# polimi-ispl/deep_prior_interpolation

Hardware: AMD Instinct MI355X
Metric: Adam iters/sec on 3D MultiRes-UNet (whole job over n_gpus; per_gpu beside it); recon SNR(dB) vs ref under config.snr_vs_reference (higher is better)
Workload: dtype f32

## Files before the change

### deep_prior_interpolation_amd/csrc/elementwise.hip

```cpp
#include "common.h"
#include <stdlib.h>

namespace {

constexpr int kStatSpan = 16384;
constexpr int kMaxStatBlocks = 2048;

__host__ __device__ inline size_t stat_span(size_t V, int nblk) {
  size_t s = (V + nblk - 1) / nblk;
  return (s + 3) & ~(size_t)3;
}

typedef float ew_f32x4 __attribute__((ext_vector_type(4)));
constexpr size_t kNtMinFloats = (size_t)32 << 20;
__device__ __forceinline__ float4 ld4(const float* p, bool nt) {
  if (nt) { const ew_f32x4 v = __builtin_nontemporal_load(reinterpret_cast<const ew_f32x4*>(p)); return make_float4(v[0], v[1], v[2], v[3]); }
  return *reinterpret_cast<const float4*>(p);
}
__device__ __forceinline__ void st4(float* p, float4 v, bool nt) {
  if (nt) __builtin_nontemporal_store((ew_f32x4){v.x, v.y, v.z, v.w}, reinterpret_cast<ew_f32x4*>(p));
  else *reinterpret_cast<float4*>(p) = v;
}

template <bool xb = false>
// ... 425 lines not shown
      const float4 t = dpi_ld4(xa, i, tb, nt);
      const float4 u = dpi_ld4(xb, i, tb, nt);
      gv[0] = g.x; gv[1] = g.y; gv[2] = g.z; gv[3] = g.w;
      av[0] = t.x; av[1] = t.y; av[2] = t.z; av[3] = t.w;
      bv[0] = u.x; bv[1] = u.y; bv[2] = u.z; bv[3] = u.w;
    } else {
#pragma unroll
      for (int j = 0; j < 4; ++j) {
        const bool in = i + j < end;
        gv[j] = in ? dpi_ld(gc, i + j, gb) : 0.f; av[j] = in ? dpi_ld(xa, i + j, tb) : 0.f; bv[j] = in ? dpi_ld(xb, i + j, tb) : 0.f;
      }
    }
    float lsf = 0.f, lqf = 0.f;
#pragma unroll
    for (int j = 0; j < 4; ++j) {
      float xh, g;
      bn_bwd_elem(ka, av[j], gv[j], xh, g);
      ra[j] = ka.a * (g - a1 - xh * a2);
      bn_bwd_elem(kb, bv[j], gv[j], xh, g);
      rb[j] = dpi_stored(kb.a * (g - b1 - xh * b2), gb);
      if (forked && i + j < end) { float h, gf_; bn_bwd_elem(kf, bv[j], rb[j], h, gf_); lsf += gf_; lqf = fmaf(gf_, h, lqf); }
    }
    if (vec) {
      dpi_st4(oa, i, make_float4(ra[0], ra[1], ra[2], ra[3]), gb, nt);
      dpi_st4(ob, i, make_float4(rb[0], rb[1], rb[2], rb[3]), gb, nt);
    } else {
      for (int j = 0; j < 4 && i + j < end; ++j) { dpi_st(oa, i + j, ra[j], gb); dpi_st(ob, i + j, rb[j], gb); }
    }
    sf += lsf; qf += lqf;
  }
  if (f_partials && f_hi > f_lo) {
    __shared__ double sh[8];
    const double SF = block_sum(sf, sh), QF = block_sum(qf, sh + 4);
    if (threadIdx.x == 0 && forked) {
      f_partials[((size_t)b * fC + fc) * 2 + 0] = SF;
      f_partials[((size_t)b * fC + fc) * 2 + 1] = QF;
    }
  }
}

template <bool fb = false>
__global__ __launch_bounds__(256) void chain_add_apply_kernel(const float* __restrict__ a, const float* __restrict__ chain_a,
                                                              const float* __restrict__ b, const float* __restrict__ chain_b,
                                                              const float* __restrict__ chain_out, size_t V, float* __restrict__ y) {
  const bool nt = (size_t)gridDim.y * V >= kNtMinFloats;
  const int c = blockIdx.y;
  const Chain ta = load_chain(chain_a, c), tb = load_chain(chain_b, c), to = load_chain(chain_out, c);
  const float* __restrict__ ac = dpi_at(a, (size_t)c * V, fb);
  const float* __restrict__ bc = dpi_at(b, (size_t)c * V, fb);
  float* __restrict__ yc = dpi_at(y, (size_t)c * V, fb);
  const bool vec = (V & 3) == 0;
  for (size_t i = ((size_t)blockIdx.x * 256 + threadIdx.x) * 4; i < V; i += (size_t)gridDim.x * 1024) {
    if (vec) {
      const float4 f = dpi_ld4(ac, i, fb, nt), g = dpi_ld4(bc, i, fb, nt);
      float4 o;
      o.x = apply_chain(to, apply_chain(ta, f.x) + apply_chain(tb, g.x)); o.y = apply_chain(to, apply_chain(ta, f.y) + apply_chain(tb, g.y));
      o.z = apply_chain(to, apply_chain(ta, f.z) + apply_chain(tb, g.z)); o.w = apply_chain(to, apply_chain(ta, f.w) + apply_chain(tb, g.w));
      dpi_st4(yc, i, o, fb, nt);
    } else {
      for (int j = 0; j < 4 && i + j < V; ++j)
        dpi_st(yc, i + j, apply_chain(to, apply_chain(ta, dpi_ld(ac, i + j, fb)) + apply_chain(tb, dpi_ld(bc, i + j, fb))), fb);
    }
  }
}

constexpr int kJoinSums = 24;
constexpr int kJoinGroups = 2;
struct JoinSide {
  const float* x;
  const float* mean_invstd;
  const float* gamma;
  const float* beta;
  const float* in_chain;
  float post;
  const float* fwd_chain;
};
struct JoinFork {
  int lo, hi;
  const float* mean_invstd;
  const float* gamma;
  const float* beta;
  float post;
};
template <bool fb = false, bool gb = false>
__global__ __launch_bounds__(256) void join_bwd_sums_kernel(const float* __restrict__ dy, const float* __restrict__ t,
                                                            const float* __restrict__ mean_invstd, const float* __restrict__ gamma,
                                                            const float* __restrict__ beta, float pre, JoinSide A, JoinSide B, JoinFork F,
                                                            int C, size_t V, int nblk, double* __restrict__ partials) {
  const bool nt = (size_t)gridDim.y * V >= kNtMinFloats;
  const int c = blockIdx.y, b = blockIdx.x;
  const BnBwd k = bn_bwd_consts(mean_invstd, gamma, beta, nullptr, pre, 1.f, C, c);
  const BnBwd ka = bn_bwd_consts(A.mean_invstd, A.gamma, A.beta, A.in_chain, 1.f, A.post, C, c);
  const BnBwd kb = bn_bwd_consts(B.mean_invstd, B.gamma, B.beta, B.in_chain, 1.f, B.post, C, c);
  const bool forked = c >= F.lo && c < F.hi;
  const int fC = F.hi - F.lo, fc = forked ? c - F.lo : 0;
  const BnBwd kf = forked ? bn_bwd_consts(F.mean_invstd, F.gamma, F.beta, nullptr, 1.f, F.post, fC, fc) : ka;
  const size_t span = stat_span(V, nblk);
  const size_t beg = (size_t)b * span, end = beg + span < V ? beg + span : V;
  const float* __restrict__ gc = dpi_at(dy, (size_t)c * V, gb);
  const float* __restrict__ tc = t ? dpi_at(t, (size_t)c * V, fb) : nullptr;
  const float* __restrict__ xa = dpi_at(A.x, (size_t)c * V, fb);
  const float* __restrict__ xb = dpi_at(B.x, (size_t)c * V, fb);
  const Chain fwa = load_chain(A.fwd_chain, c), fwb = load_chain(B.fwd_chain, c);
  double s[kJoinSums];
#pragma unroll
  for (int i = 0; i < kJoinSums; ++i) s[i] = 0.0;
  const bool vec = (V & 3) == 0;
  for (size_t i0 = beg + (size_t)threadIdx.x * 4; i0 < end; i0 += 1024 * kJoinGroups) {
   float l[kJoinSums];
#pragma unroll
   for (int q = 0; q < kJoinSums; ++q) l[q] = 0.f;
#pragma unroll
   for (int u = 0; u < kJoinGroups; ++u) {
    const size_t i = i0 + (size_t)u * 1024;
    if (i >= end) break;
    float gv[4], tv[4], av[4], bv[4];
    if (vec) {
      const float4 g = dpi_ld4(gc, i, gb, nt), p = dpi_ld4(xa, i, fb, nt), q = dpi_ld4(xb, i, fb, nt);
      gv[0] = g.x; gv[1] = g.y; gv[2] = g.z; gv[3] = g.w;
      av[0] = p.x; av[1] = p.y; av[2] = p.z; av[3] = p.w;
      bv[0] = q.x; bv[1] = q.y; bv[2] = q.z; bv[3] = q.w;
      if (tc) { const float4 u = dpi_ld4(tc, i, fb, nt); tv[0] = u.x; tv[1] = u.y; tv[2] = u.z; tv[3] = u.w; }
    } else {
#pragma unroll
      for (int j = 0; j < 4; ++j) {
        const bool in = i + j < end;
        gv[j] = in ? dpi_ld(gc, i + j, gb) : 0.f; tv[j] = (in && tc) ? dpi_ld(tc, i + j, fb) : 0.f;
        av[j] = in ? dpi_ld(xa, i + j, fb) : 0.f; bv[j] = in ? dpi_ld(xb, i + j, fb) : 0.f;
      }
    }
    if (!tc) {
#pragma unroll
      for (int j = 0; j < 4; ++j) tv[j] = apply_chain(fwa, av[j]) + apply_chain(fwb, bv[j]);
    }
#pragma unroll
    for (int j = 0; j < 4; ++j)
      if (i + j < end) {
        float X, D, Xa, ma, Xb, mb;
        bn_bwd_elem(k, tv[j], gv[j], X, D);
        bn_bwd_elem(ka, av[j], 1.f, Xa, ma);
        bn_bwd_elem(kb, bv[j], 1.f, Xb, mb);
        const float P = (k.pre == 1.f || tv[j] > 0.f) ? k.a : k.a * k.pre;
        l[0] += D; l[1] = fmaf(D, X, l[1]);
        const float wa = ma * P, wb = mb * P;
        const float waD = wa * D, waX = wa * X, wbD = wb * D, wbX = wb * X;
        l[2] += waD; l[3] += wa; l[4] += waX;
        l[5] = fmaf(waD, Xa, l[5]); l[6] = fmaf(wa, Xa, l[6]); l[7] = fmaf(waX, Xa, l[7]);
        l[8] += wbD; l[9] += wb; l[10] += wbX;
        l[11] = fmaf(wbD, Xb, l[11]); l[12] = fmaf(wb, Xb, l[12]); l[13] = fmaf(wbX, Xb, l[13]);
        if (forked) {
          float Xf, mf;
          bn_bwd_elem(kf, bv[j], 1.f, Xf, mf);
          const float wf = mf * wb, wfD = wf * D, wfX = wf * X, mfXf = mf * Xf;
          l[14] += wfD; l[15] += wf; l[16] += wfX; l[17] += mf; l[18] = fmaf(mf, Xb, l[18]);
          l[19] = fmaf(wfD, Xf, l[19]); l[20] = fmaf(wf, Xf, l[20]); l[21] = fmaf(wfX, Xf, l[21]); l[22] += mfXf; l[23] = fmaf(mfXf, Xb, l[23]);
        }
      }
   }
#pragma unroll
   for (int q = 0; q < kJoinSums; ++q) s[q] += (double)l[q];
  }
  __shared__ double sh[4][kJoinSums];
  const int lane = threadIdx.x & 63, wid = threadIdx.x >> 6;
#pragma unroll
  for (int i = 0; i < kJoinSums; ++i) {
    const double v = wave_sum(s[i]);
// ... 303 lines not shown
          reinterpret_cast<unsigned*>(reinterpret_cast<unsigned short*>(yc) + o)[0] = dpi_pack_bf16(r0, r1);
        } else {
          if (2 * w < Wo) dpi_st(yc, o, r0, yb);
          if (2 * w + 1 < Wo) dpi_st(yc, o + 1, r1, yb);
        }
      }
    }
  }
}


template <bool SCALE_D, bool gb = false>
__global__ __launch_bounds__(256) void upsample_lin_bwd_gather_kernel(const float* __restrict__ dy, int D, int H, int W, int Do, int Ho,
                                                                      int Wo, float* __restrict__ dx) {
  const int c = blockIdx.y;
  const size_t V = (size_t)D * H * W, Vo = (size_t)Do * Ho * Wo;
  const float* __restrict__ gc = dpi_at(dy, (size_t)c * Vo, gb);
  float* __restrict__ oc = dpi_at(dx, (size_t)c * V, gb);
  for (size_t i = (size_t)blockIdx.x * 256 + threadIdx.x; i < V; i += (size_t)gridDim.x * 256) {
    const int w = i % W, h = (i / W) % H, d = i / ((size_t)W * H);
    int ow[4], oh[4], od[4];
    float ww[4], wh[4], wd[4];
    lin_bwd_taps(w, W, Wo, ow, ww);
    lin_bwd_taps(h, H, Ho, oh, wh);
    if (SCALE_D) lin_bwd_taps(d, D, Do, od, wd);
    float acc = 0.f;
#pragma unroll
    for (int a = 0; a < (SCALE_D ? 4 : 1); ++a) {
      const int od_ = SCALE_D ? od[a] : d;
      const float wa = SCALE_D ? wd[a] : 1.f;
      float accd = 0.f;
#pragma unroll
      for (int b = 0; b < 4; ++b) {
        const size_t row = ((size_t)od_ * Ho + oh[b]) * Wo;
        const float rsum = ww[0] * dpi_ld(gc, row + ow[0], gb) + ww[1] * dpi_ld(gc, row + ow[1], gb) + ww[2] * dpi_ld(gc, row + ow[2], gb)
                           + ww[3] * dpi_ld(gc, row + ow[3], gb);
        accd = fmaf(wh[b], rsum, accd);
      }
      acc = fmaf(wa, accd, acc);
    }
    dpi_st(oc, i, acc, gb);
  }
}

template <bool ib = false, bool ob = false>
__global__ __launch_bounds__(256) void upsample_lin_bwd_axis_kernel(const float* __restrict__ in, float* __restrict__ out, unsigned outer,
                                                                    int n, int no, unsigned inner) {
  const unsigned slab = (unsigned)n * inner;
  const unsigned per = slab < 256 ? 256 / slab : 1;
  const unsigned sub = per > 1 ? threadIdx.x / slab : 0;
  const unsigned e = per > 1 ? threadIdx.x - sub * slab : blockIdx.x * 256 + threadIdx.x;
  if (e >= slab || sub >= per) return;
  const unsigned i = e / inner, in_i = e - i * inner;
  int oo[4];
  float wt[4];
  lin_bwd_taps((int)i, n, no, oo, wt);
  const unsigned o0 = oo[0] * inner + in_i, o1 = oo[1] * inner + in_i, o2 = oo[2] * inner + in_i, o3 = oo[3] * inner + in_i;
  for (unsigned o = blockIdx.y * per + sub; o < outer; o += gridDim.y * per) {
    const float* __restrict__ p = dpi_at(in, (size_t)o * no * inner, ib);
    dpi_st(out, (size_t)o * slab + e, (wt[0] * dpi_ld(p, o0, ib) + wt[1] * dpi_ld(p, o1, ib)) + (wt[2] * dpi_ld(p, o2, ib) + wt[3] * dpi_ld(p, o3, ib)), ob);
  }
}

__global__ __launch_bounds__(256) void upsample_lin_bwd_w2_kernel(const float* __restrict__ in, float* __restrict__ out, size_t rows, int n) {
  const int half = n >> 1, no = 2 * n;
  const size_t total = rows * (size_t)half;
  for (size_t p = (size_t)blockIdx.x * 256 + threadIdx.x; p < total; p += (size_t)gridDim.x * 256) {
    const size_t r = p / half;
    const int i = 2 * (int)(p - r * half);
    const float* __restrict__ row = in + r * no;
    const float4 v = *reinterpret_cast<const float4*>(row + 2 * i);
    const float lo = row[i > 0 ? 2 * i - 1 : 0], hi = row[i + 1 < n - 1 ? 2 * i + 4 : 0];
    int o[4];
    float w0[4], w1[4];
    lin_bwd_taps(i, n, no, o, w0);
    lin_bwd_taps(i + 1, n, no, o, w1);
    float2 y;
    y.x = (w0[0] * lo + w0[1] * v.x) + (w0[2] * v.y + w0[3] * v.z);
    y.y = (w1[0] * v.y + w1[1] * v.z) + (w1[2] * v.w + w1[3] * hi);
    *reinterpret_cast<float2*>(out + r * n + i) = y;
  }
}

__global__ __launch_bounds__(256) void crop_copy_kernel(const float* __restrict__ x, int D, int H, int W, int od, int oh, int ow,
                                                        int Do, int Ho, int Wo, float* __restrict__ y, int adjoint) {
  const int c = blockIdx.y;
  const size_t V = (size_t)D * H * W, Vo = (size_t)Do * Ho * Wo;
  if (!adjoint) {
    for (size_t i = (size_t)blockIdx.x * 256 + threadIdx.x; i < Vo; i += (size_t)gridDim.x * 256) {
      const int w = i % Wo, h = (i / Wo) % Ho, d = i / ((size_t)Wo * Ho);
      y[(size_t)c * Vo + i] = x[(size_t)c * V + ((size_t)(d + od) * H + h + oh) * W + w + ow];
    }
  } else {
    for (size_t i = (size_t)blockIdx.x * 256 + threadIdx.x; i < V; i += (size_t)gridDim.x * 256) {
      const int w = i % W, h = (i / W) % H, d = i / ((size_t)W * H);
      const int cd = d - od, ch = h - oh, cw = w - ow;
      const bool in = cd >= 0 && cd < Do && ch >= 0 && ch < Ho && cw >= 0 && cw < Wo;
      y[(size_t)c * V + i] = in ? x[(size_t)c * Vo + ((size_t)cd * Ho + ch) * Wo + cw] : 0.f;
    }
  }
}

__global__ __launch_bounds__(256) void fir_axis0_kernel(const float* __restrict__ x, const float* __restrict__ taps, int K, int T, size_t S,
                                                        float* __restrict__ y) {
  const int c = blockIdx.y, p = K / 2;
  const size_t n = (size_t)T * S;
  for (size_t i = (size_t)blockIdx.x * 256 + threadIdx.x; i < n; i += (size_t)gridDim.x * 256) {
    const int t = (int)(i / S);
    const size_t s_ = i % S;
    float acc = 0.f;
    for (int k = 0; k < K; ++k) {
      const int tt = t + p - k;
      if (tt >= 0 && tt < T) acc = fmaf(taps[k], x[(size_t)c * n + (size_t)tt * S + s_], acc);
    }
    y[(size_t)c * n + i] = acc;
  }
}

__global__ __launch_bounds__(256) void axpy_kernel(float a, const float* __restrict__ x, size_t n, float* __restrict__ y) {
  for (size_t i = (size_t)blockIdx.x * 256 + threadIdx.x; i < n; i += (size_t)gridDim.x * 256) y[i] = fmaf(a, x[i], y[i]);
}

inline unsigned ew_blocks(size_t n_vec4_threads) {
  size_t b = cdivz(n_vec4_threads, 256);
  if (b > 4096) b = 4096;
  if (b < 1) b = 1;
  return (unsigned)b;
}

}

extern "C" int dpi_stat_blocks(int C, size_t V) {
  if (C <= 0 || V == 0) return 0;
  size_t n = cdivz(V, kStatSpan);
  if (n > kMaxStatBlocks) n = kMaxStatBlocks;
  return (int)n;
}

#define DPI_LAUNCH_FG(io, KERNEL, GRID, ST, ...)                                          \
  do {                                                                                    \
    if (DPI_FB(io)) {                                                                     \
      if (DPI_GB(io)) KERNEL<true, true><<<GRID, 256, 0, ST>>>(__VA_ARGS__);              \
      else KERNEL<true, false><<<GRID, 256, 0, ST>>>(__VA_ARGS__);                        \
    } else {                                                                              \
      if (DPI_GB(io)) KERNEL<false, true><<<GRID, 256, 0, ST>>>(__VA_ARGS__);             \
      else KERNEL<false, false><<<GRID, 256, 0, ST>>>(__VA_ARGS__);                       \
    }                                                                                     \
  } while (0)
#define DPI_FB(io) (((io) & DPI_STORE_FWD_BF16) != 0)
#define DPI_GB(io) (((io) & DPI_STORE_GRAD_BF16) != 0)
#define DPI_REQUIRE_IO(io, what) DPI_REQUIRE(((io) & ~3u) == 0, what ": unknown storage-type bits in io = %u", (unsigned)(io))

extern "C" int dpi_channel_stats_io(const float* x, const float* chain, int C, size_t V, double* partials, unsigned io, void* stream) {
  DPI_REQUIRE(x && partials && C > 0 && V > 0, "channel_stats: bad argument");
  DPI_REQUIRE_IO(io, "channel_stats");
  const int nblk = dpi_stat_blocks(C, V);
  if (DPI_FB(io)) channel_stats_kernel<true><<<dim3(nblk, C), 256, 0, (hipStream_t)stream>>>(x, chain, C, V, nblk, partials);
  else channel_stats_kernel<false><<<dim3(nblk, C), 256, 0, (hipStream_t)stream>>>(x, chain, C, V, nblk, partials);
  return dpi_check_launch("channel_stats");
}
extern "C" int dpi_channel_stats(const float* x, const float* chain, int C, size_t V, double* partials, void* stream) {
  return dpi_channel_stats_io(x, chain, C, V, partials, 0, stream);
}

extern "C" int dpi_bn_finalize(const double* partials, int nblk, int C, size_t count, const float* gamma, const float* beta,
                               float eps, float momentum, float slope, int act_first, const float* in_chain, float* running_mean,
// ... 119 lines not shown
  DPI_REQUIRE(t || (fwd_chain_a && fwd_chain_b), "join_bwd: without t the two forward chains that form it are needed");
  DPI_REQUIRE(f_lo >= 0 && f_hi <= C && f_lo <= f_hi, "join_bwd: bad fork range");
  DPI_REQUIRE(f_lo == f_hi || (f_mi && dxf && dgb_f), "join_bwd: the fork range needs its BatchNorm's statistics and outputs");
  const int nblk = join_blocks(C, V);
  const JoinSide A{xa, mi_a, gamma_a, beta_a, chain_a, post_a, fwd_chain_a}, B{xb, mi_b, gamma_b, beta_b, chain_b, post_b, fwd_chain_b};
  const JoinFork F{f_lo, f_hi, f_mi, f_gamma, f_beta, f_post};
  hipStream_t st = (hipStream_t)stream;
  DPI_LAUNCH_FG(io, join_bwd_sums_kernel, dim3(nblk, C), st, dy, t, mi, gamma, beta, pre, A, B, F, C, V, nblk, ws);
  join_bwd_coef_kernel<<<C, 64, 0, st>>>(ws, nblk, C, (double)V, mi_b, gamma_b, f_lo, f_hi, coef, dgb, dgb_f);
  DPI_LAUNCH_FG(io, join_bwd_apply_kernel, dim3(ew_blocks(cdivz(V, 4 * 8)), C), st, dy, t, mi, gamma, beta, pre, A, B, F, coef, C, V, dxa, dxb, dxf);
  return dpi_check_launch("join_bwd");
}

extern "C" int dpi_chain_add_stats(const float* a, const float* chain_a, const float* b, const float* chain_b, int C, size_t V,
                                   float slope, float* t, double* partials, void* stream) {
  return dpi_chain_add_stats_io(a, chain_a, b, chain_b, C, V, slope, t, partials, 0, stream);
}
extern "C" int dpi_chain_add_stats_io(const float* a, const float* chain_a, const float* b, const float* chain_b, int C, size_t V,
                                      float slope, float* t, double* partials, unsigned io, void* stream) {
  DPI_REQUIRE(a && b && partials && C > 0 && V > 0, "chain_add_stats: bad argument");
  DPI_REQUIRE_IO(io, "chain_add_stats");
  const int nblk = dpi_stat_blocks(C, V);
  if (DPI_FB(io)) chain_add_stats_kernel<true><<<dim3(nblk, C), 256, 0, (hipStream_t)stream>>>(a, chain_a, b, chain_b, C, V, nblk, slope, t, partials);
  else chain_add_stats_kernel<false><<<dim3(nblk, C), 256, 0, (hipStream_t)stream>>>(a, chain_a, b, chain_b, C, V, nblk, slope, t, partials);
  return dpi_check_launch("chain_add_stats");
}

extern "C" int dpi_chain_add_apply(const float* a, const float* chain_a, const float* b, const float* chain_b, const float* chain_out, int C,
                                   size_t V, float* y, unsigned io, void* stream) {
  DPI_REQUIRE(a && b && y && C > 0 && V > 0, "chain_add_apply: bad argument");
  DPI_REQUIRE_IO(io, "chain_add_apply");
  if (DPI_FB(io)) chain_add_apply_kernel<true><<<dim3(ew_blocks(cdivz(V, 4)), C), 256, 0, (hipStream_t)stream>>>(a, chain_a, b, chain_b, chain_out, V, y);
  else chain_add_apply_kernel<false><<<dim3(ew_blocks(cdivz(V, 4)), C), 256, 0, (hipStream_t)stream>>>(a, chain_a, b, chain_b, chain_out, V, y);
  return dpi_check_launch("chain_add_apply");
}

extern "C" int dpi_lrelu_bwd(const float* dy, const float* x, float slope, size_t n, float* dx, void* stream) {
  DPI_REQUIRE(dy && x && dx && n > 0, "lrelu_bwd: bad argument");
  lrelu_bwd_kernel<<<ew_blocks(cdivz(n, 4)), 256, 0, (hipStream_t)stream>>>(dy, x, slope, n, dx);
  return dpi_check_launch("lrelu_bwd");
}

extern "C" int dpi_act_fwd(const float* x, size_t n, int kind, float* y, void* stream) {
  DPI_REQUIRE(x && y && n > 0 && kind >= DPI_ACT_ELU && kind <= DPI_ACT_SIGMOID, "act_fwd: bad argument");
  act_fwd_kernel<<<ew_blocks(cdivz(n, 4)), 256, 0, (hipStream_t)stream>>>(x, n, kind, y);
  return dpi_check_launch("act_fwd");
}

extern "C" int dpi_act_bwd(const float* dy, const float* y, size_t n, int kind, float* dx, void* stream) {
  DPI_REQUIRE(dy && y && dx && n > 0 && kind >= DPI_ACT_ELU && kind <= DPI_ACT_SIGMOID, "act_bwd: bad argument");
  act_bwd_kernel<<<ew_blocks(cdivz(n, 4)), 256, 0, (hipStream_t)stream>>>(dy, y, n, kind, dx);
  return dpi_check_launch("act_bwd");
}

extern "C" int dpi_add(const float* a, const float* b, size_t n, float* y, void* stream) {
  DPI_REQUIRE(a && b && y && n > 0, "add: bad argument");
  add_kernel<<<ew_blocks(cdivz(n, 4)), 256, 0, (hipStream_t)stream>>>(a, b, n, y);
  return dpi_check_launch("add");
}

extern "C" int dpi_channel_sum(const float* x, int C, size_t V, double* ws, float* out, void* stream) {
  DPI_REQUIRE(x && ws && out && C > 0 && V > 0, "channel_sum: bad argument");
  const int nblk = dpi_stat_blocks(C, V);
  channel_stats_kernel<false><<<dim3(nblk, C), 256, 0, (hipStream_t)stream>>>(x, nullptr, C, V, nblk, ws);
  if (int e = dpi_check_launch("channel_sum.stats")) return e;
  channel_sum_final_kernel<<<C, 64, 0, (hipStream_t)stream>>>(ws, nblk, C, out);
  return dpi_check_launch("channel_sum.final");
}

extern "C" int dpi_upsample2x_fwd(const float* x, const float* chain, int C, int D, int H, int W, int Do, int Ho, int Wo,
                                  int linear, float* y, void* stream) {
  return dpi_upsample2x_fwd_io(x, chain, C, D, H, W, Do, Ho, Wo, linear, y, 0, stream);
}
extern "C" int dpi_upsample2x_fwd_io(const float* x, const float* chain, int C, int D, int H, int W, int Do, int Ho, int Wo,
                                     int linear, float* y, unsigned io, void* stream) {
  DPI_REQUIRE(x && y && C > 0 && D > 0 && H > 0 && W > 0, "upsample_fwd: bad argument");
  DPI_REQUIRE_IO(io, "upsample_fwd");
  const bool fb = DPI_FB(io);
  const int scale_d = !(D == 1 && Do == 1);
  DPI_REQUIRE(Do >= 1 && Ho >= 1 && Wo >= 1 && Do <= (scale_d ? 2 * D : 1) && Ho <= 2 * H && Wo <= 2 * W,
              "upsample_fwd: output (%d,%d,%d) exceeds 2x input (%d,%d,%d)", Do, Ho, Wo, D, H, W);
  const size_t Vo = (size_t)Do * Ho * Wo, V = (size_t)D * H * W;
  if (linear && H > 1 && W > 1 && (!scale_d || D > 1)) {
    if (scale_d) {
      if (fb) upsample_lin_fwd_cube_kernel<true, true, true><<<dim3(ew_blocks(V), C), 256, 0, (hipStream_t)stream>>>(x, chain, D, H, W, Do, Ho, Wo, y);
      else upsample_lin_fwd_cube_kernel<true, false, false><<<dim3(ew_blocks(V), C), 256, 0, (hipStream_t)stream>>>(x, chain, D, H, W, Do, Ho, Wo, y);
    } else {
      if (fb) upsample_lin_fwd_cube_kernel<false, true, true><<<dim3(ew_blocks(V), C), 256, 0, (hipStream_t)stream>>>(x, chain, D, H, W, Do, Ho, Wo, y);
      else upsample_lin_fwd_cube_kernel<false, false, false><<<dim3(ew_blocks(V), C), 256, 0, (hipStream_t)stream>>>(x, chain, D, H, W, Do, Ho, Wo, y);
    }
    return dpi_check_launch("upsample_lin_fwd_cube");
  }
  if (fb) upsample_fwd_kernel<true, true><<<dim3(ew_blocks(Vo), C), 256, 0, (hipStream_t)stream>>>(x, chain, D, H, W, Do, Ho, Wo, linear, scale_d, y);
  else upsample_fwd_kernel<false, false><<<dim3(ew_blocks(Vo), C), 256, 0, (hipStream_t)stream>>>(x, chain, D, H, W, Do, Ho, Wo, linear, scale_d, y);
  return dpi_check_launch("upsample_fwd");
}

extern "C" size_t dpi_upsample2x_bwd_ws_floats(int C, int D, int H, int W, int Do, int Ho, int Wo, int linear) {
  if (!linear || C <= 0) return 0;
  const int scale_d = !(D == 1 && Do == 1);
  return (size_t)C * Do * Ho * W + (scale_d ? (size_t)C * Do * H * W : 0);
}

extern "C" int dpi_upsample2x_bwd(const float* dy, int C, int D, int H, int W, int Do, int Ho, int Wo, int linear, float* dx,
                                  float* ws, void* stream) {
  return dpi_upsample2x_bwd_io(dy, C, D, H, W, Do, Ho, Wo, linear, dx, ws, 0, stream);
}
extern "C" int dpi_upsample2x_bwd_io(const float* dy, int C, int D, int H, int W, int Do, int Ho, int Wo, int linear, float* dx,
                                     float* ws, unsigned io, void* stream) {
  DPI_REQUIRE(dy && dx && C > 0 && D > 0 && H > 0 && W > 0, "upsample_bwd: bad argument");
  DPI_REQUIRE_IO(io, "upsample_bwd");
  const bool gb = DPI_GB(io);
  const int scale_d = !(D == 1 && Do == 1);
  const size_t V = (size_t)D * H * W;
  if (linear && ws) {
    hipStream_t st = (hipStream_t)stream;
    float* t1 = ws;
    float* t2 = ws + (size_t)C * Do * Ho * W;
    DPI_REQUIRE((size_t)C * Do * Ho < (1ull << 32) && (size_t)Do * Ho * Wo < (1ull << 31) && (size_t)Do * H * W < (1ull << 31),
                "upsample_bwd: %d x %d x %d x %d exceeds the 32-bit slab indexing of the separable adjoint", C, Do, Ho, Wo);
    auto launch = [&](const float* src, float* dst, size_t outer, int n, int no, size_t inner, bool ib, bool ob) {
      const unsigned gx = (unsigned)cdivz((size_t)n * inner, 256);
      size_t gy = outer < 65535 ? outer : 65535;
      while (gy > 1 && (size_t)gx * gy > 16384) gy = (gy + 1) / 2;
      const dim3 g(gx, (unsigned)gy);
      if (ib && ob) upsample_lin_bwd_axis_kernel<true, true><<<g, 256, 0, st>>>(src, dst, (unsigned)outer, n, no, (unsigned)inner);
      else if (ib) upsample_lin_bwd_axis_kernel<true, false><<<g, 256, 0, st>>>(src, dst, (unsigned)outer, n, no, (unsigned)inner);
      else if (ob) upsample_lin_bwd_axis_kernel<false, true><<<g, 256, 0, st>>>(src, dst, (unsigned)outer, n, no, (unsigned)inner);
      else upsample_lin_bwd_axis_kernel<false, false><<<g, 256, 0, st>>>(src, dst, (unsigned)outer, n, no, (unsigned)inner);
    };
    static const bool w2 = getenv("DPI_NO_UPW2") == nullptr;
    if (w2 && !gb && Wo == 2 * W && (W & 1) == 0 && (Wo & 3) == 0 && (((uintptr_t)dy | (uintptr_t)t1) & 15) == 0) {
      const size_t rows = (size_t)C * Do * Ho, pairs = rows * (size_t)(W / 2);
      upsample_lin_bwd_w2_kernel<<<ew_blocks(cdivz(pairs, 1)), 256, 0, st>>>(dy, t1, rows, W);
    } else
    launch(dy, t1, (size_t)C * Do * Ho, W, Wo, 1, gb, false);
    launch(t1, scale_d ? t2 : dx, (size_t)C * Do, H, Ho, W, false, scale_d ? false : gb);
    if (scale_d) launch(t2, dx, C, D, Do, (size_t)H * W, false, gb);
    return dpi_check_launch("upsample_lin_bwd_axis");
  }
  if (linear) {
    if (scale_d) {
      if (gb) upsample_lin_bwd_gather_kernel<true, true><<<dim3(ew_blocks(V), C), 256, 0, (hipStream_t)stream>>>(dy, D, H, W, Do, Ho, Wo, dx);
      else upsample_lin_bwd_gather_kernel<true, false><<<dim3(ew_blocks(V), C), 256, 0, (hipStream_t)stream>>>(dy, D, H, W, Do, Ho, Wo, dx);
    } else {
      if (gb) upsample_lin_bwd_gather_kernel<false, true><<<dim3(ew_blocks(V), C), 256, 0, (hipStream_t)stream>>>(dy, D, H, W, Do, Ho, Wo, dx);
      else upsample_lin_bwd_gather_kernel<false, false><<<dim3(ew_blocks(V), C), 256, 0, (hipStream_t)stream>>>(dy, D, H, W, Do, Ho, Wo, dx);
    }
    return dpi_check_launch("upsample_lin_bwd_gather");
  }
  if (gb) upsample_bwd_kernel<true><<<dim3(ew_blocks(V), C), 256, 0, (hipStream_t)stream>>>(dy, D, H, W, Do, Ho, Wo, linear, scale_d, dx);
  else upsample_bwd_kernel<false><<<dim3(ew_blocks(V), C), 256, 0, (hipStream_t)stream>>>(dy, D, H, W, Do, Ho, Wo, linear, scale_d, dx);
  return dpi_check_launch("upsample_bwd");
}

extern "C" int dpi_crop_copy(const float* x, int C, int D, int H, int W, int od, int oh, int ow, int Do, int Ho, int Wo, float* y,
                             void* stream) {
  DPI_REQUIRE(x && y && od >= 0 && oh >= 0 && ow >= 0 && od + Do <= D && oh + Ho <= H && ow + Wo <= W, "crop_copy: bad window");
  crop_copy_kernel<<<dim3(ew_blocks((size_t)Do * Ho * Wo), C), 256, 0, (hipStream_t)stream>>>(x, D, H, W, od, oh, ow, Do, Ho, Wo,
                                                                                            y, 0);
  return dpi_check_launch("crop_copy");
}

extern "C" int dpi_crop_copy_bwd(const float* dy, int C, int D, int H, int W, int od, int oh, int ow, int Do, int Ho, int Wo,
                                 float* dx, void* stream) {
  DPI_REQUIRE(dy && dx && od >= 0 && oh >= 0 && ow >= 0 && od + Do <= D && oh + Ho <= H && ow + Wo <= W, "crop_copy_bwd: bad window");
  crop_copy_kernel<<<dim3(ew_blocks((size_t)D * H * W), C), 256, 0, (hipStream_t)stream>>>(dy, D, H, W, od, oh, ow, Do, Ho, Wo, dx,
                                                                                         1);
  return dpi_check_launch("crop_copy_bwd");
}

extern "C" int dpi_fir_axis0(const float* x, const float* taps, int K, int C, int T, size_t S, float* y, void* stream) {
  DPI_REQUIRE(x && taps && y && K > 0 && (K & 1) && C > 0 && T > 0 && S > 0, "fir_axis0: bad argument (odd tap count required)");
  fir_axis0_kernel<<<dim3(ew_blocks((size_t)T * S), C), 256, 0, (hipStream_t)stream>>>(x, taps, K, T, S, y);
  return dpi_check_launch("fir_axis0");
}

extern "C" int dpi_axpy(float a, const float* x, size_t n, float* y, void* stream) {
  DPI_REQUIRE(x && y && n > 0, "axpy: bad argument");
  axpy_kernel<<<ew_blocks(n), 256, 0, (hipStream_t)stream>>>(a, x, n, y);
  return dpi_check_launch("axpy");
}
```

Before: 33.88.

## Add LDS-tiled trilinear upsample forward and fused separable backward kernels

Adds shared-memory tiled kernels for 2x linear upsampling. The forward kernel stages a haloed input tile in LDS and emits float4 outputs computed separably from it. The backward kernel fuses the three separable adjoint passes into one launch: it does the W-axis pass with wave shuffles into LDS, then the H and D passes, which removes the workspace round trips through global memory. The cost is extra LDS use, halo recomputation at tile edges, and new fast paths that apply only when shapes and pointers are aligned.

New measurement: 34.31 (median of 6 runs). No clear change (+1.3%).

```diff
diff --git a/deep_prior_interpolation_amd/csrc/elementwise.hip b/deep_prior_interpolation_amd/csrc/elementwise.hip
--- a/deep_prior_interpolation_amd/csrc/elementwise.hip
+++ b/deep_prior_interpolation_amd/csrc/elementwise.hip
@@ -531,6 +531,8 @@
   const float* beta;
   float post;
 };
+typedef dpi_f32x2 ew_f2;
+__device__ __forceinline__ ew_f2 splat2(float v) { return (ew_f2){v, v}; }
 template <bool fb = false, bool gb = false>
 __global__ __launch_bounds__(256) void join_bwd_sums_kernel(const float* __restrict__ dy, const float* __restrict__ t,
                                                             const float* __restrict__ mean_invstd, const float* __restrict__ gamma,
@@ -1000,6 +1002,155 @@
   }
 }
 
+template <bool SCALE_D, int TD, int TH, int TW>
+__global__ __launch_bounds__(256) void upsample_lin_fwd_tile_kernel(const float* __restrict__ x, const float* __restrict__ chain, int D, int H,
+                                                                    int W, int Do, int Ho, int nth, int ntw, float* __restrict__ y) {
+  constexpr int LD = SCALE_D ? TD + 2 : 1, LH = TH + 2, LW = TW + 2, PW = TW / 2;
+  __shared__ __attribute__((aligned(16))) float tile[LD * LH * LW];
+  const int c = blockIdx.y, Wo = 2 * W;
+  const size_t V = (size_t)D * H * W, Vo = (size_t)Do * Ho * Wo;
+  const bool nt = (size_t)gridDim.y * Vo >= kNtMinFloats;
+  const int tw_i = blockIdx.x % ntw, th_i = (blockIdx.x / ntw) % nth, td_i = blockIdx.x / (ntw * nth);
+  const int d0 = td_i * TD, h0 = th_i * TH, w0 = tw_i * TW;
+  const Chain t = load_chain(chain, c);
+  const float* __restrict__ xc = x + (size_t)c * V;
+  float* __restrict__ yc = y + (size_t)c * Vo;
+#pragma unroll
+  for (int e = threadIdx.x; e < LD * LH * LW; e += 256) {
+    const int lw = e % LW, lh = (e / LW) % LH, ld = e / (LW * LH);
+    const int d = SCALE_D ? min(max(d0 + ld - 1, 0), D - 1) : 0;
+    const int h = min(max(h0 + lh - 1, 0), H - 1), w = min(max(w0 + lw - 1, 0), W - 1);
+    tile[e] = apply_chain(t, xc[((size_t)d * H + h) * W + w]);
+  }
+  __syncthreads();
+  for (int it = threadIdx.x; it < TD * TH * PW; it += 256) {
+    const int pw = it % PW, lh = (it / PW) % TH, ld = it / (PW * TH);
+    const int d = d0 + ld, h = h0 + lh, w = w0 + 2 * pw;
+    if (d >= D || h >= H || w >= W) continue;
+    ew_f2 wv[3][3][2];
+#pragma unroll
+    for (int a = 0; a < (SCALE_D ? 3 : 1); ++a)
+#pragma unroll
+      for (int b = 0; b < 3; ++b) {
+        const float* __restrict__ r = tile + ((SCALE_D ? ld + a : 0) * LH + lh + b) * LW + 2 * pw;
+        const float2 p = *reinterpret_cast<const float2*>(r), q = *reinterpret_cast<const float2*>(r + 2);
+        const float v0 = p.x, v1 = p.y, v2 = q.x, v3 = q.y;
+        wv[a][b][0] = (ew_f2){.25f * v0 + .75f * v1, .75f * v1 + .25f * v2};
+        wv[a][b][1] = (ew_f2){.25f * v1 + .75f * v2, .75f * v2 + .25f * v3};
+      }
+    const ew_f2 q4 = splat2(.25f), t4 = splat2(.75f);
+#pragma unroll
+    for (int oh_ = 0; oh_ < 2; ++oh_) {
+      const int oh = 2 * h + oh_;
+      if (oh >= Ho) continue;
+      ew_f2 hv[3][2];
+#pragma unroll
+      for (int a = 0; a < (SCALE_D ? 3 : 1); ++a)
+#pragma unroll
+        for (int j = 0; j < 2; ++j) hv[a][j] = oh_ == 0 ? q4 * wv[a][0][j] + t4 * wv[a][1][j] : t4 * wv[a][1][j] + q4 * wv[a][2][j];
+#pragma unroll
+      for (int od_ = 0; od_ < (SCALE_D ? 2 : 1); ++od_) {
+        const int od = SCALE_D ? 2 * d + od_ : d;
+        if (od >= Do) continue;
+        ew_f2 r[2];
+#pragma unroll
+        for (int j = 0; j < 2; ++j) r[j] = !SCALE_D ? hv[0][j] : od_ == 0 ? q4 * hv[0][j] + t4 * hv[1][j] : t4 * hv[1][j] + q4 * hv[2][j];
+        st4(yc + ((size_t)od * Ho + oh) * Wo + 2 * w, make_float4(r[0].x, r[0].y, r[1].x, r[1].y), nt);
+      }
+    }
+  }
+}
+
+template <bool SCALE_D, int TD, int TH, int TW>
+__global__ __launch_bounds__(256) void upsample_lin_bwd_tile_kernel(const float* __restrict__ dy, int D, int H, int W, int Do, int Ho, int nth,
+                                                                    int ntw, float* __restrict__ dx) {
+  constexpr int PD = SCALE_D ? 2 * TD + 2 : 1, PH = 2 * TH + 2, PW = TW / 2;
+  __shared__ __attribute__((aligned(16))) float tile[PD * PH * TW];
+  const int c = blockIdx.y, Wo = 2 * W;
+  const size_t V = (size_t)D * H * W, Vo = (size_t)Do * Ho * Wo;
+  const int tw_i = blockIdx.x % ntw, th_i = (blockIdx.x / ntw) % nth, td_i = blockIdx.x / (ntw * nth);
+  const int d0 = td_i * TD, h0 = th_i * TH, w0 = tw_i * TW;
+  const float* __restrict__ gc = dy + (size_t)c * Vo;
+  float* __restrict__ oc = dx + (size_t)c * V;
+  constexpr int NB = 4;
+  static_assert(64 % PW == 0, "a tile row must not straddle two waves");
+  for (int e0 = threadIdx.x; e0 - (int)threadIdx.x < PD * PH * PW; e0 += 256 * NB) {
+    float4 v[NB];
+    float lo[NB], hi[NB];
+#pragma unroll
+    for (int u = 0; u < NB; ++u) {
+      const int e = e0 + u * 256;
+      const int pw = e % PW, ph = (e / PW) % PH, pd = e / (PW * PH);
+      const int i = w0 + 2 * pw;
+      const bool ok = e < PD * PH * PW && i < W;
+      int od = SCALE_D ? 2 * d0 - 1 + pd : 0, oh = 2 * h0 - 1 + ph;
+      if (od < 0 || od >= Do) od = 0;
+      if (oh < 0 || oh >= Ho) oh = 0;
+      const float* __restrict__ row = gc + ((size_t)od * Ho + oh) * Wo;
+      v[u] = make_float4(0.f, 0.f, 0.f, 0.f);
+      if (ok) v[u] = *reinterpret_cast<const float4*>(row + 2 * i);
+    }
+#pragma unroll
+    for (int u = 0; u < NB; ++u) {
+      const int e = e0 + u * 256;
+      const int pw = e % PW, ph = (e / PW) % PH, pd = e / (PW * PH);
+      const int i = w0 + 2 * pw;
+      const bool ok = e < PD * PH * PW && i < W;
+      int od = SCALE_D ? 2 * d0 - 1 + pd : 0, oh = 2 * h0 - 1 + ph;
+      if (od < 0 || od >= Do) od = 0;
+      if (oh < 0 || oh >= Ho) oh = 0;
+      const float* __restrict__ row = gc + ((size_t)od * Ho + oh) * Wo;
+      const float up = __shfl_up(v[u].w, 1, 64), dn = __shfl_down(v[u].x, 1, 64);
+      const bool lo_lane = pw > 0, hi_lane = pw < PW - 1 && i + 2 < W;
+      lo[u] = up; hi[u] = dn;
+      if (ok && !lo_lane) lo[u] = row[i > 0 ? 2 * i - 1 : 0];
+      if (ok && !hi_lane) hi[u] = row[i + 1 < W - 1 ? 2 * i + 4 : 0];
+    }
+#pragma unroll
+    for (int u = 0; u < NB; ++u) {
+      const int e = e0 + u * 256;
+      const int pw = e % PW, ph = (e / PW) % PH, pd = e / (PW * PH);
+      const int i = w0 + 2 * pw;
+      if (e >= PD * PH * PW || i >= W) continue;
+      int o[4];
+      float u0[4], u1[4];
+      lin_bwd_taps(i, W, Wo, o, u0);
+      lin_bwd_taps(i + 1, W, Wo, o, u1);
+      float2 s;
+      s.x = (u0[0] * lo[u] + u0[1] * v[u].x) + (u0[2] * v[u].y + u0[3] * v[u].z);
+      s.y = (u1[0] * v[u].y + u1[1] * v[u].z) + (u1[2] * v[u].w + u1[3] * hi[u]);
+      *reinterpret_cast<float2*>(tile + (pd * PH + ph) * TW + 2 * pw) = s;
+    }
+  }
+  __syncthreads();
+  for (int it = threadIdx.x; it < TD * TH * TW; it += 256) {
+    const int lw = it % TW, lh = (it / TW) % TH, ld = it / (TW * TH);
+    const int d = d0 + ld, h = h0 + lh, w = w0 + lw;
+    if (d >= D || h >= H || w >= W) continue;
+    int o[4];
+    float wh[4], wd[4];
+    lin_bwd_taps(h, H, Ho, o, wh);
+    float hs[4];
+#pragma unroll
+    for (int a = 0; a < (SCALE_D ? 4 : 1); ++a) {
+      const float* __restrict__ p = tile + ((SCALE_D ? 2 * ld + a : 0) * PH + 2 * lh) * TW + lw;
+      hs[a] = (wh[0] * p[0] + wh[1] * p[TW]) + (wh[2] * p[2 * TW] + wh[3] * p[3 * TW]);
+    }
+    float r = hs[0];
+    if (SCALE_D) {
+      lin_bwd_taps(d, D, Do, o, wd);
+      r = (wd[0] * hs[0] + wd[1] * hs[1]) + (wd[2] * hs[2] + wd[3] * hs[3]);
+    }
+    oc[((size_t)d * H + h) * W + w] = r;
+  }
+}
+
+template <bool SCALE_D, int TD, int TH, int TW>
+static void launch_upsample_bwd_tile(const float* dy, int C, int D, int H, int W, int Do, int Ho, float* dx, hipStream_t st) {
+  const int ntd = cdiv(D, TD), nth = cdiv(H, TH), ntw = cdiv(W, TW);
+  upsample_lin_bwd_tile_kernel<SCALE_D, TD, TH, TW><<<dim3((unsigned)(ntd * nth * ntw), C), 256, 0, st>>>(dy, D, H, W, Do, Ho, nth, ntw, dx);
+}
+
 __global__ __launch_bounds__(256) void crop_copy_kernel(const float* __restrict__ x, int D, int H, int W, int od, int oh, int ow,
                                                         int Do, int Ho, int Wo, float* __restrict__ y, int adjoint) {
   const int c = blockIdx.y;
@@ -1285,6 +1436,17 @@
               "upsample_fwd: output (%d,%d,%d) exceeds 2x input (%d,%d,%d)", Do, Ho, Wo, D, H, W);
   const size_t Vo = (size_t)Do * Ho * Wo, V = (size_t)D * H * W;
   if (linear && H > 1 && W > 1 && (!scale_d || D > 1)) {
+    if (!fb && Wo == 2 * W && (W & 1) == 0 && ((uintptr_t)y & 15) == 0 && C <= 65535) {
+      hipStream_t st = (hipStream_t)stream;
+      if (scale_d) {
+        const int nth = cdiv(H, 8), ntw = cdiv(W, 32);
+        upsample_lin_fwd_tile_kernel<true, 4, 8, 32><<<dim3((unsigned)(cdiv(D, 4) * nth * ntw), C), 256, 0, st>>>(x, chain, D, H, W, Do, Ho, nth, ntw, y);
+      } else {
+        const int nth = cdiv(H, 16), ntw = cdiv(W, 32);
+        upsample_lin_fwd_tile_kernel<false, 1, 16, 32><<<dim3((unsigned)(nth * ntw), C), 256, 0, st>>>(x, chain, D, H, W, Do, Ho, nth, ntw, y);
+      }
+      return dpi_check_launch("upsample_lin_fwd_tile");
+    }
     if (scale_d) {
       if (fb) upsample_lin_fwd_cube_kernel<true, true, true><<<dim3(ew_blocks(V), C), 256, 0, (hipStream_t)stream>>>(x, chain, D, H, W, Do, Ho, Wo, y);
       else upsample_lin_fwd_cube_kernel<true, false, false><<<dim3(ew_blocks(V), C), 256, 0, (hipStream_t)stream>>>(x, chain, D, H, W, Do, Ho, Wo, y);
@@ -1318,6 +1480,17 @@
   const size_t V = (size_t)D * H * W;
   if (linear && ws) {
     hipStream_t st = (hipStream_t)stream;
+    if (!gb && Wo == 2 * W && (W & 1) == 0 && ((uintptr_t)dy & 15) == 0 && C <= 65535) {
+      if (scale_d) {
+        if (W > 32) launch_upsample_bwd_tile<true, 4, 8, 64>(dy, C, D, H, W, Do, Ho, dx, st);
+        else if (W > 16) launch_upsample_bwd_tile<true, 4, 16, 32>(dy, C, D, H, W, Do, Ho, dx, st);
+        else launch_upsample_bwd_tile<true, 4, 32, 16>(dy, C, D, H, W, Do, Ho, dx, st);
+      } else {
+        if (W > 32) launch_upsample_bwd_tile<false, 1, 16, 64>(dy, C, D, H, W, Do, Ho, dx, st);
+        else launch_upsample_bwd_tile<false, 1, 32, 32>(dy, C, D, H, W, Do, Ho, dx, st);
+      }
+      return dpi_check_launch("upsample_lin_bwd_tile");
+    }
     float* t1 = ws;
     float* t2 = ws + (size_t)C * Do * Ho * W;
     DPI_REQUIRE((size_t)C * Do * Ho < (1ull << 32) && (size_t)Do * Ho * Wo < (1ull << 31) && (size_t)Do * H * W < (1ull << 31),
```
